# multiplefish/VPLines-SLAM

Hardware: AMD Instinct MI355X
Metric: sliding-window BA solves/sec (10 KF, 200 pts + 80 lines, 5 iters) (higher is better)
Workload: dtype f64

## Files before the change

vplines-slam_amd/csrc/ba_common.h:

```cpp
#pragma once
#include <hip/hip_runtime.h>
#include "ba_types.h"
#include "ba_asm_pattern.h"
#include "vpl_math.h"

namespace vpl {

#ifdef VPL_STAMPS
#define VPL_STAMP(B, w, i) do { if (threadIdx.x == 0) (B).dbg[(size_t)(w) * 64 + (i)] = (long long)__builtin_readcyclecounter(); } while (0)
#define VPL_IVAL(acc) long long acc = 0
#define VPL_IVAL_START(t) long long t = __builtin_readcyclecounter()
#define VPL_IVAL_ADD(acc, t) acc += __builtin_readcyclecounter() - (t)
#define VPL_IVAL_LAP(acc, t) do { const long long now_ = __builtin_readcyclecounter(); acc += now_ - (t); t = now_; } while (0)
#define VPL_IVAL_STORE(cond, dst, ...) do { long long* dst_ = (dst); if (dst_ && (cond)) { const long long v_[] = {__VA_ARGS__}; \
  for (int i_ = 0; i_ < (int)(sizeof(v_) / sizeof(v_[0])); ++i_) dst_[i_] = v_[i_]; } } while (0)
#else
#define VPL_STAMP(B, w, i) do {} while (0)
#define VPL_IVAL(acc) do {} while (0)
#define VPL_IVAL_START(t) do {} while (0)
#define VPL_IVAL_ADD(acc, t) do {} while (0)
#define VPL_IVAL_LAP(acc, t) do {} while (0)
#define VPL_IVAL_STORE(cond, dst, ...) do {} while (0)
#endif

__device__ __forceinline__ void count_active(const DevBatch& B, int k) {
  if (B.act && threadIdx.x == 0 && B.launch < ACT_SLOTS) atomicAdd(&B.act[4 * B.launch + k], 1);
}

__device__ __forceinline__ int ordered_window(const DevBatch& B) {
  const int w = B.ord_it == 0 ? (int)blockIdx.x : B.order[(size_t)(B.ord_it & 1) * B.nW + blockIdx.x];
  return __builtin_amdgcn_readfirstlane(w);
}

__device__ __forceinline__ double wave_sum(double v) {
#pragma unroll
  for (int o = 32; o > 0; o >>= 1) v += __shfl_xor(v, o, 64);
  return v;
}

template <int CTRL>
__device__ __forceinline__ double dpp_shr_f64(double v) {
  const int lo = __builtin_amdgcn_update_dpp(0, __double2loint(v), CTRL, 0xf, 0xf, true);
  const int hi = __builtin_amdgcn_update_dpp(0, __double2hiint(v), CTRL, 0xf, 0xf, true);
  return __hiloint2double(hi, lo);
}
__device__ __forceinline__ double row_sum16(double v) {
  v += dpp_shr_f64<0x111>(v);
  v += dpp_shr_f64<0x112>(v);
  v += dpp_shr_f64<0x114>(v);
  v += dpp_shr_f64<0x118>(v);
// ... 145 lines not shown
```

vplines-slam_amd/csrc/ba_limits.h:

```cpp
#pragma once

namespace vpl {

constexpr int NF = 11;
constexpr int NC = 171;
constexpr int NV = 72;
constexpr int MAXKEEP = 80;

}
```

vplines-slam_amd/csrc/ba_lin.h:

```cpp
#pragma once
#include "ba_common.h"

namespace vpl {

typedef double v4d_lin __attribute__((ext_vector_type(4)));
constexpr int LIN_THREADS = 512;
constexpr int STG_LD = 17;
constexpr int LIN_STAGE = 8 * 32 * STG_LD;
constexpr int PRE_LDS = 62;
constexpr int LIN_HW = 720;
constexpr int PREP_NMAX = 112;
__host__ __device__ constexpr int lin_stage_doubles(int maxL) {
  const int ln = 8 * LIN_HW + 38 * maxL;
  const int pt = LIN_STAGE + 78 * 36 + NV;
  const int m = ln > pt ? ln : pt;
  return m > 4650 + 3570 ? m : 4650 + 3570;
}
constexpr int PREP_THREADS = 640;
inline size_t prep_smem(int max_prior_n) {
  const int ns = max_prior_n < PREP_NMAX ? max_prior_n : PREP_NMAX;
  return (size_t)((PREP_THREADS / 64) * 675 + ns * ns + ns + 84) * sizeof(double);
}
constexpr size_t PREP_SMEM = (size_t)((PREP_THREADS / 64) * 675 + PREP_NMAX * PREP_NMAX + PREP_NMAX + 84) * sizeof(double);

// ... 388 lines not shown
        for (int c2 = 0; c2 <= a; ++c2, ++t) { Hl[4 * a + c2] = la[t]; Hl[4 * c2 + a] = la[t]; }
#pragma unroll
        for (int c2 = 0; c2 < 6; ++c2) B.Wl[(li * 4 + a) * WS + WS - 6 + c2] = la[14 + 6 * a + c2];
      }
    }
  }
  for (int e = tid; e < LIN_HW; e += T) {
    double v = 0.0;
#pragma unroll
    for (int q = 0; q < 8; ++q) v += lin_ln_Hw(imuJ, q)[e];
    if (e < 693) {
      const int f = e / 63, q = e - 63 * f;
      if (q < 21) {
        int a, c2;
        tri_decode(q, a, c2);
        Hv[hvi(6 * f + a, 6 * f + c2)] += v;
      } else if (q < 57) {
        const int a = (q - 21) / 6, c2 = (q - 21) % 6;
        Hv[hvi(66 + a, 6 * f + c2)] += v;
      } else {
        gv[6 * f + (q - 57)] += v;
      }
    } else if (e < 714) {
      int a, c2;
      tri_decode(e - 693, a, c2);
      Hv[hvi(66 + a, 66 + c2)] += v;
    } else {
      gv[66 + (e - 714)] += v;
    }
  }
}

template <int MODE>
__device__ __forceinline__ void lin_imu_raw(const DevBatch& B, const int w, const double* xp, const double* xs, const double* plds, double* imuJ, double* imur,
                                               int* imuact, double (&sa)[2][4]) {
  constexpr bool MARG = MODE != 0;
  constexpr bool PRIOR_ONLY = MODE == 2;
  const int tid = threadIdx.x, T = LIN_THREADS, lane = tid & 63;
  for (int i = tid; i < 4650; i += T) imuJ[i] = 0.0;
#pragma unroll
  for (int q = 0; q < 2; ++q) {
    const int f = (tid >> 6) + 8 * q;
    const double* S = B.pre[(size_t)w * NF + (f < 10 ? f : 0) + 1].sqrt_info;
#pragma unroll
    for (int ks = 0; ks < 4; ++ks) {
      const int k = 4 * ks + (lane >> 4), i = lane & 15;
      sa[q][ks] = (f < 10 && i < 15 && k < 15 && k >= i) ? S[i * 15 + k] : 0.0;
    }
  }
  __syncthreads();
  if ((tid & 63) < 10 && tid < 128) {
    const int f = tid & 63, j = f + 1;
    const DevPreint& dp = *(const DevPreint*)(plds + PRE_LDS * f);
    bool act = MARG ? (j == 1 && dp.sum_dt < 10.0) : !(dp.sum_dt > 10.0);
    if (PRIOR_ONLY) act = false;
    if (tid < 64) imuact[f] = act ? 1 : 0;
    if (act) {
      PreInt p = load_preint(dp);
      if (tid < 64) {
        imu_residual_raw(p, xp + 7 * (j - 1), xs + 9 * (j - 1), xp + 7 * j, xs + 9 * j, B.opt.g_norm, imur + 15 * f);
      } else {
        ImuJac JB = imu_jacobian_raw(p, xp + 7 * (j - 1), xs + 9 * (j - 1), xp + 7 * j, xs + 9 * j, B.opt.g_norm);
        imu_jac_dense(JB, imuJ + 450 * f);
      }
    }
  }
}
__device__ __forceinline__ void lin_asm_request(const DevBatch& B, int2 (&asmd)[LIN_ASM_PER_THREAD]) {
  const int tid = threadIdx.x, T = LIN_THREADS;
#pragma unroll
  for (int u = 0; u < LIN_ASM_PER_THREAD; ++u) {
    const int i = u * T + tid;
    asmd[u] = ((const int2*)B.asm_tab)[i < NZ_N ? i : 0];
  }
}
__device__ __forceinline__ void lin_imu_whiten(double* imuJ, double* imur, const int* imuact, const double (&sa)[2][4]) {
  const int tid = threadIdx.x, T = LIN_THREADS, lane = tid & 63;
  double* imuH = lin_imuH(imuJ);
  const int wvi = tid >> 6, m16 = lane & 15, kk = lane >> 4;
  v4d_lin cd[2] = {{0, 0, 0, 0}, {0, 0, 0, 0}};
  for (int i = tid; i < 120; i += T) imuH[i] = 0.0;
#pragma unroll
  for (int q = 0; q < 2; ++q) {
    const int f = wvi + 8 * q;
    if (f >= 10) break;
    double* J = imuJ + 450 * f;
    double* rr = imur + 15 * f;
    const bool on = imuact[f] != 0;
    v4d_lin jw[2] = {{0, 0, 0, 0}, {0, 0, 0, 0}};
#pragma unroll
    for (int ct = 0; ct < 2; ++ct) {
      const int c = 16 * ct + m16;
#pragma unroll
      for (int ks = 0; ks < 4; ++ks) {
        const int k = 4 * ks + kk;
        const double bv = k < 15 ? (c < 30 ? J[k * 30 + c] : (c == 30 ? rr[k] : 0.0)) : 0.0;
        jw[ct] = __builtin_amdgcn_mfma_f64_16x16x4f64(on ? sa[q][ks] : 0.0, bv, jw[ct], 0, 0, 0);
      }
    }
    __builtin_amdgcn_wave_barrier();
    if (on) {
#pragma unroll
      for (int ct = 0; ct < 2; ++ct) {
        const double vals[4] = {jw[ct].x, jw[ct].y, jw[ct].z, jw[ct].w};
        const int c = 16 * ct + m16;
#pragma unroll
        for (int v = 0; v < 4; ++v) {
          const int r = kk + 4 * v;
          if (r < 15) {
            if (c < 30) J[r * 30 + c] = vals[v];
            else if (c == 30) rr[r] = vals[v];
          }
        }
      }
    }
    __builtin_amdgcn_fence(__ATOMIC_RELEASE, "workgroup");
    __builtin_amdgcn_wave_barrier();
    __builtin_amdgcn_fence(__ATOMIC_ACQUIRE, "workgroup");
    v4d_lin c00 = {0, 0, 0, 0}, c10 = {0, 0, 0, 0}, c11 = {0, 0, 0, 0};
#pragma unroll
    for (int ks = 0; ks < 4; ++ks) {
      const int k = 4 * ks + kk;
      const double lo = k < 15 ? J[k * 30 + m16] : 0.0;
      const double hi = (k < 15 && m16 < 14) ? J[k * 30 + 16 + m16] : 0.0;
      c00 = __builtin_amdgcn_mfma_f64_16x16x4f64(lo, lo, c00, 0, 0, 0);
      c10 = __builtin_amdgcn_mfma_f64_16x16x4f64(hi, lo, c10, 0, 0, 0);
      c11 = __builtin_amdgcn_mfma_f64_16x16x4f64(hi, hi, c11, 0, 0, 0);
    }
    {
      const double v00[4] = {c00.x, c00.y, c00.z, c00.w}, v10[4] = {c10.x, c10.y, c10.z, c10.w}, v11[4] = {c11.x, c11.y, c11.z, c11.w};
      double keep[4] = {0, 0, 0, 0};
#pragma unroll
      for (int v = 0; v < 4; ++v) {
        const int i0 = kk + 4 * v, j0 = m16;
        if (i0 < 15 && j0 < 15) keep[v] = v00[v];
        const int i1 = 16 + kk + 4 * v;
        if (i1 < 30) {
          if (j0 < 15) imuH[11 * 120 + 225 * f + 15 * (i1 - 15) + j0] = v10[v];
          else imuH[120 * (f + 1) + (i1 - 15) * (i1 - 14) / 2 + 0] = v10[v];
          const int j1 = 16 + m16;
          if (j1 < 30 && j1 <= i1) imuH[120 * (f + 1) + (i1 - 15) * (i1 - 14) / 2 + (j1 - 15)] = v11[v];
        }
        if (i0 == 15) {
          if (j0 < 15) imuH[11 * 120 + 225 * f + j0] = v00[v];
          else imuH[120 * (f + 1)] = v00[v];
        }
      }
      cd[q] = v4d_lin{keep[0], keep[1], keep[2], keep[3]};
    }
  }
  __syncthreads();
#pragma unroll
  for (int q = 0; q < 2; ++q) {
    const int f = wvi + 8 * q;
    if (f >= 10) break;
    const double keep[4] = {cd[q].x, cd[q].y, cd[q].z, cd[q].w};
#pragma unroll
    for (int v = 0; v < 4; ++v) {
      const int i0 = kk + 4 * v, j0 = m16;
      if (i0 < 15 && j0 <= i0) imuH[120 * f + i0 * (i0 + 1) / 2 + j0] += keep[v];
    }
  }
}
__device__ __forceinline__ void lin_imu_cost(const double* imur, const int* imuact, double& cost) {
  const int tid = threadIdx.x;
  if (tid < 10 && imuact[tid]) {
    double s = 0;
    for (int k = 0; k < 15; ++k) s += imur[15 * tid + k] * imur[15 * tid + k];
    cost += 0.5 * s;
  }
}

__device__ __forceinline__ void lin_handover_in(const DevBatch& B, const int w, double* sm, double& cost) {
  const int tid = threadIdx.x, T = LIN_THREADS;
  if (tid == 0) {
    while (__hip_atomic_load(&B.lin_flag[w], __ATOMIC_RELAXED, __HIP_MEMORY_SCOPE_AGENT) != 1) __builtin_amdgcn_s_sleep(32);
    __hip_atomic_store(&B.lin_flag[w], 0, __ATOMIC_RELAXED, __HIP_MEMORY_SCOPE_AGENT);
  }
  __syncthreads();
  const double* part = B.lin_part + (size_t)w * LIN_PART;
  for (int i = tid; i < HV_DOUBLES + NV; i += T) sm[i] += __hip_atomic_load(&part[i], __ATOMIC_RELAXED, __HIP_MEMORY_SCOPE_AGENT);
  if (tid == 0) cost += __hip_atomic_load(&part[HV_DOUBLES + NV], __ATOMIC_RELAXED, __HIP_MEMORY_SCOPE_AGENT);
  __syncthreads();
}

__device__ __forceinline__ void lin_asm_store(const int2 d, const double* Hv, const double* imuH, const double* prH, const int* invmap,
                                                 const bool prior_lds, const bool ex_free, double* Hout) {
  const int hv = d.x & 0xffff, im = d.x >> 16, r = d.y & 255, c = (d.y >> 8) & 255, e = d.y >> 16;
  const double vh = Hv[hv ? hv - 1 : 0], vi = imuH[im ? im - 1 : 0];
  const int ir = prior_lds ? invmap[r] : -1, ic = prior_lds ? invmap[c] : -1;
  const bool hp = ir >= 0 && ic >= 0;
  const int hi_ = ic > ir ? ic : ir, lo_ = ic > ir ? ir : ic;
  const double vp = prH[hp ? hi_ * (hi_ + 1) / 2 + lo_ : 0];
  double v = hv ? vh : 0.0;
  v += im ? vi : 0.0;
// ... 439 lines not shown
          for (int a = 0; a < 6; ++a) {
            if (a >= c0) {
              const double gev = row_sum16(Je[a] * r[0] + Je[6 + a] * r[1]);
              if (leader) lds_add(&Hw[714 + a], gev);
            }
#pragma unroll
            for (int c2 = 0; c2 <= a; ++c2, ++t) {
              if (a < c0 || c2 < c0) continue;
              const double v = row_sum16(Je[a] * Je[c2] + Je[6 + a] * Je[6 + c2]);
              if (leader) lds_add(&Hw[693 + t], v);
            }
          }
        }
      }
      if (act) {
        double* Wl = B.Wl + li * 4 * WS;
#pragma unroll
        for (int a = 0; a < 4; ++a)
#pragma unroll
          for (int c2 = 0; c2 < 6; ++c2) Wl[a * WS + 6 * k + c2] = Wj[6 * a + c2];
      }
    }
  }
  __syncthreads();
  lin_lines_out(B, w, Hv, gv, imuJ, nL);
  __syncthreads();
  VPL_STAMP(B, w, 25);
  double sa[2][4];
  lin_imu_raw<MODE>(B, w, xp, xs, plds, imuJ, imur, imuact, sa);
  __syncthreads();
  VPL_STAMP(B, w, 28);
  int2 asmd[LIN_ASM_PER_THREAD];
  lin_asm_request(B, asmd);
  lin_imu_whiten(imuJ, imur, imuact, sa);
  __syncthreads();
  lin_imu_cost(imur, imuact, cost);
  if (ROLE == 2) {
    lin_handover_in(B, w, sm, cost);
  } else if (!MARG) {
    if (tid == 0) cost += cost_pts;
  }
  VPL_STAMP(B, w, 20);
  lin_assemble(B, w, Hv, gv, imuJ, imur, prg, prH, PRH_N, invmap, imuact, P.n, ex_free, asmd);
  VPL_STAMP(B, w, 21);
  lin_finish<MODE>(tr, red, cost);
}
template <int MODE>
__global__ __launch_bounds__(LIN_THREADS) void k_lin(DevBatch B) {
  extern __shared__ double sm[];
  lin_body<MODE, 0>(B, MODE == 0 ? ordered_window(B) : (int)blockIdx.x, sm);
}
__global__ __launch_bounds__(LIN_THREADS) void k_lin2(DevBatch B) {
  extern __shared__ double sm[];
  const int nlin = B.ord_it == 0 ? B.nW : B.ord_cnt[2 * (B.ord_it & 1)];
  if (2 * nlin > B.ncu) {
    if ((int)blockIdx.x < B.nW) lin_body<0, 0>(B, ordered_window(B), sm);
    return;
  }
  const int b = (int)(blockIdx.x >> 4) * 8 + (int)(blockIdx.x & 7);
  if (b >= B.nW) return;
  const int w = __builtin_amdgcn_readfirstlane(B.ord_it == 0 ? b : B.order[(size_t)(B.ord_it & 1) * B.nW + b]);
  if (blockIdx.x & 8) lin_body<0, 2>(B, w, sm);
  else lin_body<0, 1>(B, w, sm);
}

constexpr size_t LIN_LDS_BUDGET = 158 * 1024;
inline size_t lin_smem_base(int maxP, int maxL) {
// ... 17 lines not shown
```

vplines-slam_amd/csrc/vpl_math.h:

```cpp
#pragma once
#include <math.h>

#ifdef __HIPCC__
#define VPL_HD __host__ __device__ __forceinline__
#else
#define VPL_HD inline
#endif

namespace vpl {

struct V3 {
  double x, y, z;
};
struct M3 {
  double m[9];
};

VPL_HD V3 v3(double x, double y, double z) { return V3{x, y, z}; }
VPL_HD V3 operator+(V3 a, V3 b) { return V3{a.x + b.x, a.y + b.y, a.z + b.z}; }
VPL_HD V3 operator-(V3 a, V3 b) { return V3{a.x - b.x, a.y - b.y, a.z - b.z}; }
VPL_HD V3 operator-(V3 a) { return V3{-a.x, -a.y, -a.z}; }
VPL_HD V3 operator*(V3 a, double s) { return V3{a.x * s, a.y * s, a.z * s}; }
VPL_HD V3 operator*(double s, V3 a) { return V3{a.x * s, a.y * s, a.z * s}; }
VPL_HD double dot(V3 a, V3 b) { return a.x * b.x + a.y * b.y + a.z * b.z; }
// ... 393 lines not shown
};
VPL_HD void imu_residual_raw(const PreInt& p, const double* pi, const double* sbi, const double* pj, const double* sbj,
                             double g_norm, double* r) {
  V3 Pi{pi[0], pi[1], pi[2]}, Pj{pj[0], pj[1], pj[2]};
  Q4 Qi = qpose(pi), Qj = qpose(pj);
  V3 Vi{sbi[0], sbi[1], sbi[2]}, Bai{sbi[3], sbi[4], sbi[5]}, Bgi{sbi[6], sbi[7], sbi[8]};
  V3 Vj{sbj[0], sbj[1], sbj[2]}, Baj{sbj[3], sbj[4], sbj[5]}, Bgj{sbj[6], sbj[7], sbj[8]};
  V3 G{0, 0, g_norm};
  V3 dba = Bai - p.lba, dbg = Bgi - p.lbg;
  Q4 cq = qmul(p.dq, deltaQ(mul(p.dq_dbg, dbg)));
  V3 cv = p.dv + mul(p.dv_dba, dba) + mul(p.dv_dbg, dbg);
  V3 cp = p.dp + mul(p.dp_dba, dba) + mul(p.dp_dbg, dbg);
  double dt = p.sum_dt;
  Q4 Qii = qinv(Qi);
  V3 rp = qrot(Qii, G * (0.5 * dt * dt) + Pj - Pi - Vi * dt) - cp;
  Q4 qe = qmul(qinv(cq), qmul(Qii, Qj));
  V3 rq{2 * qe.x, 2 * qe.y, 2 * qe.z};
  V3 rv = qrot(Qii, G * dt + Vj - Vi) - cv;
  V3 rba = Baj - Bai, rbg = Bgj - Bgi;
  r[0] = rp.x; r[1] = rp.y; r[2] = rp.z; r[3] = rq.x; r[4] = rq.y; r[5] = rq.z;
  r[6] = rv.x; r[7] = rv.y; r[8] = rv.z; r[9] = rba.x; r[10] = rba.y; r[11] = rba.z;
  r[12] = rbg.x; r[13] = rbg.y; r[14] = rbg.z;
}
VPL_HD M3 qleft_br(Q4 q) {
  M3 S = skew(V3{q.x, q.y, q.z});
  S.m[0] += q.w; S.m[4] += q.w; S.m[8] += q.w;
  return S;
}
VPL_HD M3 qright_br(Q4 q) {
  M3 S = skew(V3{-q.x, -q.y, -q.z});
  S.m[0] += q.w; S.m[4] += q.w; S.m[8] += q.w;
  return S;
}
struct ImuJac {
  M3 pi_pp, pi_pr, pi_rr, pi_vr;
  M3 si_pv, si_pba, si_pbg, si_rbg, si_vv, si_vba, si_vbg;
  M3 pj_pp, pj_rr;
  M3 sj_vv;
};
VPL_HD M3 neg(const M3& A) {
  M3 C;
#pragma unroll
  for (int k = 0; k < 9; ++k) C.m[k] = -A.m[k];
  return C;
}
VPL_HD M3 scale(const M3& A, double s) {
  M3 C;
#pragma unroll
  for (int k = 0; k < 9; ++k) C.m[k] = A.m[k] * s;
  return C;
}
VPL_HD ImuJac imu_jacobian_raw(const PreInt& p, const double* pi, const double* sbi, const double* pj,
                               const double* sbj, double g_norm) {
  V3 Pi{pi[0], pi[1], pi[2]}, Pj{pj[0], pj[1], pj[2]};
  Q4 Qi = qpose(pi), Qj = qpose(pj);
  V3 Vi{sbi[0], sbi[1], sbi[2]}, Bgi{sbi[6], sbi[7], sbi[8]};
  V3 Vj{sbj[0], sbj[1], sbj[2]};
  V3 G{0, 0, g_norm};
  double dt = p.sum_dt;
  Q4 Qii = qinv(Qi);
  M3 RiT = qmat(Qii);
  Q4 cq = qmul(p.dq, deltaQ(mul(p.dq_dbg, Bgi - p.lbg)));
  ImuJac J;
  J.pi_pp = neg(RiT);
  J.pi_pr = skew(qrot(Qii, G * (0.5 * dt * dt) + Pj - Pi - Vi * dt));
  {
    Q4 ql = qmul(qinv(Qj), Qi);
    M3 A = qleft_br(ql), B = qright_br(cq);
    M3 AB = mul(A, B);
    V3 vl{ql.x, ql.y, ql.z}, vr{cq.x, cq.y, cq.z};
    double vlv[3] = {vl.x, vl.y, vl.z}, vrv[3] = {vr.x, vr.y, vr.z};
#pragma unroll
    for (int i = 0; i < 3; ++i)
#pragma unroll
      for (int j = 0; j < 3; ++j) AB.m[3 * i + j] += -vlv[i] * vrv[j];
    J.pi_rr = neg(AB);
  }
  J.pi_vr = skew(qrot(Qii, G * dt + Vj - Vi));
  J.si_pv = scale(RiT, -dt);
  J.si_pba = neg(p.dp_dba);
  J.si_pbg = neg(p.dp_dbg);
  J.si_rbg = neg(mul(qleft_br(qmul(qmul(qinv(Qj), Qi), cq)), p.dq_dbg));
  J.si_vv = neg(RiT);
  J.si_vba = neg(p.dv_dba);
  J.si_vbg = neg(p.dv_dbg);
  J.pj_pp = RiT;
  J.pj_rr = qleft_br(qmul(qmul(qinv(cq), Qii), Qj));
  J.sj_vv = RiT;
  return J;
}
VPL_HD void put33(double* J, int ld, int r0, int c0, const M3& B) {
#pragma unroll
  for (int i = 0; i < 3; ++i)
#pragma unroll
    for (int j = 0; j < 3; ++j) J[(r0 + i) * ld + c0 + j] = B.m[3 * i + j];
}
VPL_HD void imu_jac_dense(const ImuJac& B, double* J ) {
  put33(J, 30, 0, 0, B.pi_pp); put33(J, 30, 0, 3, B.pi_pr); put33(J, 30, 3, 3, B.pi_rr); put33(J, 30, 6, 3, B.pi_vr);
  put33(J, 30, 0, 6, B.si_pv); put33(J, 30, 0, 9, B.si_pba); put33(J, 30, 0, 12, B.si_pbg);
  put33(J, 30, 3, 12, B.si_rbg);
  put33(J, 30, 6, 6, B.si_vv); put33(J, 30, 6, 9, B.si_vba); put33(J, 30, 6, 12, B.si_vbg);
  J[9 * 30 + 9] = -1; J[10 * 30 + 10] = -1; J[11 * 30 + 11] = -1;
  J[12 * 30 + 12] = -1; J[13 * 30 + 13] = -1; J[14 * 30 + 14] = -1;
  put33(J, 30, 0, 15, B.pj_pp); put33(J, 30, 3, 18, B.pj_rr);
  put33(J, 30, 6, 21, B.sj_vv);
  J[9 * 30 + 24] = 1; J[10 * 30 + 25] = 1; J[11 * 30 + 26] = 1;
  J[12 * 30 + 27] = 1; J[13 * 30 + 28] = 1; J[14 * 30 + 29] = 1;
}

}
```

vplines-slam_amd/csrc/vplines_ba.hip:

```cpp
#include <hip/hip_runtime.h>

#include <algorithm>
#include <chrono>
#include <memory>
#include <cstdlib>
#include <cstring>
#include <string>
#include <vector>

#include "vplines_ba.h"
#include "ba_types.h"
#include "ba_lin.h"
#include "ba_pack.h"
#include "ba_solve.h"
#include "ba_step.h"
#include "ba_marg.h"
#include "ba_prior_eig.h"
#include "ba_lineopt.h"
#include "ba_factors.h"
#include "ba_odo.h"
#include "odo_tracks.h"
#include "host_common.h"

using namespace vpl;
// ... 87 lines not shown
  {
    int ncu = 0;
    if (hipDeviceGetAttribute(&ncu, hipDeviceAttributeMultiprocessorCount, device) != hipSuccess || ncu <= 0) ncu = 256;
    if (const char* sv = std::getenv("VPL_BA_LIN_SPLIT")) ncu = std::atoi(sv) ? 1 << 30 : 0;
    B.ncu = ncu;
  }
  B.maxPR = max_point_unit_rounds(B.maxP, B.maxPO);
  B.maxKS = max_schur_ksteps(B.maxP, B.maxL);
  B.llSlots = line_lane_slots(B.maxL);
  const size_t W = max_windows;
  hipError_t e = hipSuccess;
#define AL(ptr, n) if (e == hipSuccess) e = dalloc(c, &B.ptr, (size_t)(n))
  AL(pose, W * 77); AL(sb, W * 99); AL(ex, W * 7); AL(invd, W * B.maxP); AL(orth, W * B.maxL * 4);
  AL(pose_c, W * 77); AL(sb_c, W * 99); AL(ex_c, W * 7); AL(invd_c, W * B.maxP); AL(orth_c, W * B.maxL * 4); AL(lw, W * B.maxL * 6); AL(lw_c, W * B.maxL * 6);
  AL(lin_part, W * LIN_PART); AL(lin_pcost, W); AL(lin_flag, W);
  AL(pose_0, W * 77); AL(sb_0, W * 99); AL(ex_0, W * 7); AL(invd_0, W * B.maxP); AL(plk_0, W * B.maxL * 6);
  AL(plk, W * B.maxL * 6); AL(gauge, W * 4); AL(fail_ref, W * 13); AL(orth_in, W);
  AL(nP, W); AL(nL, W);
  AL(pt_start, W * B.maxP); AL(pt_nobs, W * B.maxP); AL(pt_off, W * B.maxP); AL(pt_obs, W * B.maxPO * 3);
  AL(ps_list, W * B.maxP); AL(ps_cnt, W * (NF + 1)); AL(pu_lane, W * B.maxPR * 1024); AL(pu_sub, W * B.maxPR * 512); AL(pu_cnt, W); AL(pu_cnt0, W);
  AL(ln_start, W * B.maxL); AL(ln_nobs, W * B.maxL); AL(ln_off, W * B.maxL); AL(ln_obs, W * B.maxLO * 8);
  AL(nLO, W); AL(lo_ln, W * B.maxLO);
  AL(ll_tab, W * B.llSlots * 2); AL(ll_np, W);
  AL(pre, W * NF);
  AL(pr_n, W); AL(pr_nb, W); AL(pr_kind, W * MAXPB); AL(pr_frame, W * MAXPB); AL(pr_idx, W * MAXPB);
  AL(pr_x0, W * MAXPB * 9); AL(pr_J0, W * MAXPN * MAXPN); AL(pr_r0, W * MAXPN); AL(pr_H, W * MAXPN * MAXPN); AL(pr_g0, W * MAXPN);
  AL(pr_map, W * MAXPN);
  AL(Hcc, W * NCP); AL(gc, W * NC); AL(asm_tab, 2 * NCP); AL(Hpp, W * B.maxP); AL(gp, W * B.maxP); AL(Wp, W * B.maxP * NV);
  AL(Hll, W * B.maxL * 16); AL(gl, W * B.maxL * 4); AL(Wl, W * B.maxL * 4 * NV); AL(lchol, W * B.maxL * 10);
  AL(tr, W);
  AL(scale, W * B.nfull); AL(diag, W * B.nfull); AL(grad, W * B.nfull); AL(gn, W * B.nfull);
  AL(mg_n, W); AL(mg_nb, W); AL(mg_kind, W * MAXPB); AL(mg_frame, W * MAXPB); AL(mg_idx, W * MAXPB);
  AL(mg_cam, W * MAXPB); AL(mg_x0, W * MAXPB * 9); AL(mg_J0, W * MAXKEEP * MAXKEEP); AL(mg_r0, W * MAXKEEP);
  AL(mg_A, W * MAXKEEP * MAXKEEP); AL(mg_b, W * MAXKEEP); AL(mg_m, W); AL(dbg, W * 64); AL(ln_removed, W * B.maxL); AL(ln_tri, W * B.maxL);
  if (e == hipSuccess) e = dalloc(c, &c->d_act, (size_t)ACT_SLOTS * 4);
  AL(order, 2 * W); AL(ord_cnt, 4);
  AL(sk_tab, W * B.maxKS * 4); AL(sk_wave, W * 8 * SK_WSTRIDE); AL(sacc, W * SACC_N); AL(nz_tab, NZ_N); AL(ycs, W * 176); AL(sx, W * 8); AL(path, W);
#undef AL
  if (e != hipSuccess) return VPL_E_HIP;
  if (lin_smem_base(c->maxP, c->maxL) > LIN_LDS_BUDGET) return VPL_E_CAPACITY;
  B.prhN = lin_prh_n(c->maxP, c->maxL);
  {
    std::vector<int> nz, tab;
    asm_build_tables(nz, tab);
    if ((int)nz.size() != NZ_N || (int)tab.size() != 2 * NCP) return VPL_E_HIP;
    if (hipMemcpy(B.asm_tab, tab.data(), tab.size() * sizeof(int), hipMemcpyHostToDevice) != hipSuccess) return VPL_E_HIP;
    if (hipMemcpy(B.nz_tab, nz.data(), nz.size() * sizeof(int), hipMemcpyHostToDevice) != hipSuccess) return VPL_E_HIP;
  }
  static size_t lin_max = 0, solve_max = 0, schur_max = 0, back_max = 0, step_max = 0;
  lin_max = std::max(lin_max, lin_smem(c->maxP, c->maxL));
  solve_max = std::max(solve_max, solve_smem(c->maxP, c->maxL));
  schur_max = std::max(schur_max, schur_smem(c->maxP, c->maxL));
  back_max = std::max(back_max, back_smem(c->maxP, c->maxL));
  step_max = std::max(step_max, step_smem(c->maxP, c->maxL));
  if (schur_max > 159 * 1024 || back_max > 159 * 1024) return VPL_E_CAPACITY;
  const std::pair<const void*, size_t> lds[] = {
      {(const void*)k_lin2, lin_max}, {(const void*)k_lin<1>, lin_max}, {(const void*)k_lin<2>, lin_max},
      {(const void*)k_solve, solve_max}, {(const void*)k_schur<3>, schur_max}, {(const void*)k_schur<5>, schur_max},
      {(const void*)k_schur_mixed, schur_max}, {(const void*)k_chol, chol_smem()}, {(const void*)k_back, back_max},
      {(const void*)k_step<3, false>, step_max}, {(const void*)k_step<3, true>, step_max}, {(const void*)k_step<5, false>, step_max},
      {(const void*)k_prep, PREP_SMEM}, {(const void*)k_marg<MARG_THREADS>, MARG_LDS_MAX}, {(const void*)k_marg<256>, MARG_LDS_SMALL},
      {(const void*)k_prior_eigen, prior_eig_layout(MAXKEEP).bytes}, {(const void*)k_init_align, init_lds_bytes(INIT_NMAX)}};
  for (const auto& k : lds)
    if (hipFuncSetAttribute(k.first, hipFuncAttributeMaxDynamicSharedMemorySize, (int)k.second) != hipSuccess) return VPL_E_HIP;
  vpl_ba_default_options(&c->opt);
  if (const char* gv = std::getenv("VPL_BA_GRAPH")) c->use_graph = std::atoi(gv) != 0;
  if (const char* gv = std::getenv("VPL_BA_GENERAL")) c->force_general = std::atoi(gv) != 0;
// ... 921 lines not shown
  HIPCHK(c, dat.alloc(N * 8)); HIPCHK(c, drt.alloc(N * 8)); HIPCHK(c, drank.alloc(N * 4)); HIPCHK(c, dperm.alloc(N * MAXKEEP * 4));
  HIPCHK(c, dJ.alloc(N * M2 * 8)); HIPCHK(c, dr.alloc(N * MAXKEEP * 8));
  HIPCHK(c, hipMemcpyAsync(dn.p, n, N * 4, hipMemcpyHostToDevice, c->stream));
  HIPCHK(c, hipMemcpyAsync(dA.p, A, N * M2 * 8, hipMemcpyHostToDevice, c->stream));
  HIPCHK(c, hipMemcpyAsync(db.p, b, N * MAXKEEP * 8, hipMemcpyHostToDevice, c->stream));
  HIPCHK(c, hipMemcpyAsync(dat.p, abs_tol, N * 8, hipMemcpyHostToDevice, c->stream));
  HIPCHK(c, hipMemcpyAsync(drt.p, rel_tol, N * 8, hipMemcpyHostToDevice, c->stream));
  HIPCHK(c, hipMemsetAsync(drank.p, 0xff, N * 4, c->stream));
  HIPCHK(c, hipMemsetAsync(dperm.p, 0xff, N * MAXKEEP * 4, c->stream));
  HIPCHK(c, hipMemsetAsync(dJ.p, 0xff, N * M2 * 8, c->stream));
  HIPCHK(c, hipMemsetAsync(dr.p, 0xff, N * MAXKEEP * 8, c->stream));
  const size_t smem = (size_t)psd_test_lds_doubles(nmax) * sizeof(double);
  const void* kern = threads == 256 ? (const void*)k_psd_factor<256> : (const void*)k_psd_factor<512>;
  HIPCHK(c, hipFuncSetAttribute(kern, hipFuncAttributeMaxDynamicSharedMemorySize, psd_test_lds_doubles(MAXKEEP) * (int)sizeof(double)));
  if (threads == 256)
    hipLaunchKernelGGL(k_psd_factor<256>, dim3(n_cases), dim3(256), smem, c->stream, form, (const int*)dn.p, dA.d(), db.d(), dat.d(),
                       drt.d(), (int*)drank.p, (int*)dperm.p, dJ.d(), dr.d());
  else
    hipLaunchKernelGGL(k_psd_factor<512>, dim3(n_cases), dim3(512), smem, c->stream, form, (const int*)dn.p, dA.d(), db.d(), dat.d(),
                       drt.d(), (int*)drank.p, (int*)dperm.p, dJ.d(), dr.d());
  HIPCHK(c, hipGetLastError());
  HIPCHK(c, hipMemcpyAsync(rank, drank.p, N * 4, hipMemcpyDeviceToHost, c->stream));
  HIPCHK(c, hipMemcpyAsync(perm, dperm.p, N * MAXKEEP * 4, hipMemcpyDeviceToHost, c->stream));
  HIPCHK(c, hipMemcpyAsync(J0, dJ.p, N * M2 * 8, hipMemcpyDeviceToHost, c->stream));
  HIPCHK(c, hipMemcpyAsync(r0, dr.p, N * MAXKEEP * 8, hipMemcpyDeviceToHost, c->stream));
  HIPCHK(c, hipStreamSynchronize(c->stream));
  return VPL_OK;
}

int vpl_ba_debug_guards(vpl_ctx* c) { return debug_guards(c); }
int vpl_ba_debug_allocs(vpl_ctx* c, long long* n_arrays, long long* payload_bytes) { return debug_allocs(c, n_arrays, payload_bytes); }

int vpl_ba_debug_stamps(vpl_ctx* c, int w, long long* out) {
  HIPCHK(c, hipMemcpy(out, c->B.dbg + (size_t)w * 64, 64 * 8, hipMemcpyDeviceToHost));
  return VPL_OK;
}

int vpl_ba_debug_point_units(int n_points, const int* point_start, const int* point_nobs, int max_rounds, int* lane_table,
                             int* unit_table, int* rounds, int* rounds0) {
  if (n_points < 0 || !point_start || !point_nobs || !lane_table || !unit_table || !rounds || !rounds0 || max_rounds < 1) return VPL_E_INVALID;
  std::vector<int> off(n_points + 1, 0), list(n_points + 1, 0);
  int cnt[NF + 1];
  int o = 0;
  for (int p = 0; p < n_points; ++p) {
    if (point_start[p] < 0 || point_nobs[p] < 2 || point_start[p] + point_nobs[p] > NF) return VPL_E_INVALID;
    off[p] = o; o += point_nobs[p];
  }
  sort_points_by_start(n_points, point_start, point_nobs, list.data(), cnt);
  PointUnitLayout PL;
  if (!pack_point_units(point_nobs, off.data(), list.data(), cnt, max_rounds, lane_table, unit_table, &PL)) return VPL_E_CAPACITY;
  *rounds = PL.rounds; *rounds0 = PL.rounds0;
  return VPL_OK;
}
int vpl_ba_debug_point_chains(const int* unit_table, int rounds, int rounds0, int marg_pass) {
  if (!unit_table || rounds < 0 || rounds0 < 0 || rounds0 > rounds) return VPL_E_INVALID;
  PointUnitLayout PL;
  PL.rounds = rounds; PL.rounds0 = rounds0;
  return point_unit_chains_finish(unit_table, PL, marg_pass != 0) ? 1 : 0;
}

int vpl_ba_enable_kernel_timing(vpl_ctx* c, int enable) {
  if (!c) return VPL_E_INVALID;
  c->timing = enable != 0;
  c->ktimes.clear();
  return VPL_OK;
}
int vpl_ba_kernel_times(vpl_ctx* c, int* count, const char** names, double* total_ms, int* launches) {
// ... 34 lines not shown
```

Measured before the change: 273,800.

## Split IMU Jacobian into per-wave groups and rebalance IMU whitening across waves

Splits the IMU Jacobian computation into four independent block groups, each computed by a different wave alongside the residual wave, instead of one thread per frame computing the whole Jacobian. It also reorganises IMU whitening and Gram products so that eight waves each own one frame and the remaining frames are dealt out across waves by tile. Zeroing of the IMU Hessian is restricted to inactive frames. The intent is to shorten the serial per-thread Jacobian latency and balance MFMA work across waves, at the cost of recomputing shared quaternion terms in each group and adding an extra block barrier. Extra debug stamp slots are added as well.

```diff
diff --git a/vplines-slam_amd/csrc/ba_common.h b/vplines-slam_amd/csrc/ba_common.h
--- a/vplines-slam_amd/csrc/ba_common.h
+++ b/vplines-slam_amd/csrc/ba_common.h
@@ -7,7 +7,8 @@
 namespace vpl {
 
 #ifdef VPL_STAMPS
-#define VPL_STAMP(B, w, i) do { if (threadIdx.x == 0) (B).dbg[(size_t)(w) * 64 + (i)] = (long long)__builtin_readcyclecounter(); } while (0)
+#define VPL_STAMP_T(B, w, i, t) do { if (threadIdx.x == (t)) (B).dbg[(size_t)(w) * DBG_SLOTS + (i)] = (long long)__builtin_readcyclecounter(); } while (0)
+#define VPL_STAMP(B, w, i) VPL_STAMP_T(B, w, i, 0)
 #define VPL_IVAL(acc) long long acc = 0
 #define VPL_IVAL_START(t) long long t = __builtin_readcyclecounter()
 #define VPL_IVAL_ADD(acc, t) acc += __builtin_readcyclecounter() - (t)
@@ -16,6 +17,7 @@
   for (int i_ = 0; i_ < (int)(sizeof(v_) / sizeof(v_[0])); ++i_) dst_[i_] = v_[i_]; } } while (0)
 #else
 #define VPL_STAMP(B, w, i) do {} while (0)
+#define VPL_STAMP_T(B, w, i, t) do {} while (0)
 #define VPL_IVAL(acc) do {} while (0)
 #define VPL_IVAL_START(t) do {} while (0)
 #define VPL_IVAL_ADD(acc, t) do {} while (0)
diff --git a/vplines-slam_amd/csrc/ba_limits.h b/vplines-slam_amd/csrc/ba_limits.h
--- a/vplines-slam_amd/csrc/ba_limits.h
+++ b/vplines-slam_amd/csrc/ba_limits.h
@@ -5,6 +5,7 @@
 constexpr int NF = 11;
 constexpr int NC = 171;
 constexpr int NV = 72;
+constexpr int DBG_SLOTS = 80;
 constexpr int MAXKEEP = 80;
 
 }
diff --git a/vplines-slam_amd/csrc/ba_lin.h b/vplines-slam_amd/csrc/ba_lin.h
--- a/vplines-slam_amd/csrc/ba_lin.h
+++ b/vplines-slam_amd/csrc/ba_lin.h
@@ -444,39 +444,60 @@
 }
 
 template <int MODE>
+__device__ __forceinline__ bool lin_imu_active(const double* plds, const int f) {
+  const DevPreint& dp = *(const DevPreint*)(plds + PRE_LDS * f);
+  if (MODE == 2) return false;
+  return MODE != 0 ? (f == 0 && dp.sum_dt < 10.0) : !(dp.sum_dt > 10.0);
+}
+template <int MODE>
+struct LinImuDeal {
+  static constexpr int OWN = MODE == 0 ? 8 : 0;
+  static constexpr int DEALT = MODE == 0 ? 2 : (MODE == 1 ? 1 : 0);
+};
+template <int MODE>
+__device__ __forceinline__ void lin_imu_request(const DevBatch& B, const int w, const double* plds, const int q, const int wvi, double (&sa)[4]) {
+  using D = LinImuDeal<MODE>;
+  const int lane = threadIdx.x & 63;
+  const int f = q == 0 ? wvi : D::OWN + (wvi >> 1);
+  const bool have = q == 0 ? wvi < D::OWN : wvi < 2 * D::DEALT;
+  const bool on = have && lin_imu_active<MODE>(plds, have ? f : 0);
+  const double* S = B.pre[(size_t)w * NF + (have ? f : 0) + 1].sqrt_info;
+#pragma unroll
+  for (int ks = 0; ks < 4; ++ks) {
+    const int k = 4 * ks + (lane >> 4), i = lane & 15;
+    sa[ks] = (on && i < 15 && k < 15 && k >= i) ? S[i * 15 + k] : 0.0;
+  }
+}
+template <int MODE>
 __device__ __forceinline__ void lin_imu_raw(const DevBatch& B, const int w, const double* xp, const double* xs, const double* plds, double* imuJ, double* imur,
                                                int* imuact, double (&sa)[2][4]) {
-  constexpr bool MARG = MODE != 0;
-  constexpr bool PRIOR_ONLY = MODE == 2;
   const int tid = threadIdx.x, T = LIN_THREADS, lane = tid & 63;
+  const int wvi = __builtin_amdgcn_readfirstlane(tid >> 6);
   for (int i = tid; i < 4650; i += T) imuJ[i] = 0.0;
-#pragma unroll
-  for (int q = 0; q < 2; ++q) {
-    const int f = (tid >> 6) + 8 * q;
-    const double* S = B.pre[(size_t)w * NF + (f < 10 ? f : 0) + 1].sqrt_info;
-#pragma unroll
-    for (int ks = 0; ks < 4; ++ks) {
-      const int k = 4 * ks + (lane >> 4), i = lane & 15;
-      sa[q][ks] = (f < 10 && i < 15 && k < 15 && k >= i) ? S[i * 15 + k] : 0.0;
-    }
-  }
-  __syncthreads();
-  if ((tid & 63) < 10 && tid < 128) {
-    const int f = tid & 63, j = f + 1;
-    const DevPreint& dp = *(const DevPreint*)(plds + PRE_LDS * f);
-    bool act = MARG ? (j == 1 && dp.sum_dt < 10.0) : !(dp.sum_dt > 10.0);
-    if (PRIOR_ONLY) act = false;
-    if (tid < 64) imuact[f] = act ? 1 : 0;
+  lin_imu_request<MODE>(B, w, plds, 0, wvi, sa[0]);
+  lin_imu_request<MODE>(B, w, plds, 1, wvi, sa[1]);
+  __syncthreads();
+  VPL_STAMP(B, w, 64);
+  if (lane < 10 && wvi < 5) {
+    const int f = lane, j = f + 1;
+    const bool act = lin_imu_active<MODE>(plds, f);
+    if (wvi == 0) imuact[f] = act ? 1 : 0;
     if (act) {
-      PreInt p = load_preint(dp);
-      if (tid < 64) {
-        imu_residual_raw(p, xp + 7 * (j - 1), xs + 9 * (j - 1), xp + 7 * j, xs + 9 * j, B.opt.g_norm, imur + 15 * f);
-      } else {
-        ImuJac JB = imu_jacobian_raw(p, xp + 7 * (j - 1), xs + 9 * (j - 1), xp + 7 * j, xs + 9 * j, B.opt.g_norm);
-        imu_jac_dense(JB, imuJ + 450 * f);
-      }
-    }
-  }
+      const DevPreint& dp = *(const DevPreint*)(plds + PRE_LDS * f);
+      const double *pi = xp + 7 * (j - 1), *sbi = xs + 9 * (j - 1), *pj = xp + 7 * j, *sbj = xs + 9 * j;
+      const double g_norm = B.opt.g_norm;
+      if (wvi == 0) { const PreInt p = load_preint(dp); imu_residual_raw(p, pi, sbi, pj, sbj, g_norm, imur + 15 * f); }
+      else if (wvi == 1) { const PreInt p = load_preint(dp); imu_jac_group_dense(0, p, pi, sbi, pj, sbj, g_norm, imuJ + 450 * f); }
+      else if (wvi == 2) { const PreInt p = load_preint(dp); imu_jac_group_dense(1, p, pi, sbi, pj, sbj, g_norm, imuJ + 450 * f); }
+      else if (wvi == 3) { const PreInt p = load_preint(dp); imu_jac_group_dense(2, p, pi, sbi, pj, sbj, g_norm, imuJ + 450 * f); }
+      else { const PreInt p = load_preint(dp); imu_jac_group_dense(3, p, pi, sbi, pj, sbj, g_norm, imuJ + 450 * f); }
+    }
+  }
+  VPL_STAMP(B, w, 65);
+  VPL_STAMP_T(B, w, 72, 64);
+  VPL_STAMP_T(B, w, 73, 128);
+  VPL_STAMP_T(B, w, 74, 192);
+  VPL_STAMP_T(B, w, 75, 256);
 }
 __device__ __forceinline__ void lin_asm_request(const DevBatch& B, int2 (&asmd)[LIN_ASM_PER_THREAD]) {
   const int tid = threadIdx.x, T = LIN_THREADS;
@@ -486,46 +507,89 @@
     asmd[u] = ((const int2*)B.asm_tab)[i < NZ_N ? i : 0];
   }
 }
-__device__ __forceinline__ void lin_imu_whiten(double* imuJ, double* imur, const int* imuact, const double (&sa)[2][4]) {
+__device__ __forceinline__ v4d_lin lin_imu_whiten_tile(const double* J, const double* rr, const double (&sa)[4], const int ct, const int m16, const int kk) {
+  v4d_lin jw = {0, 0, 0, 0};
+  const int c = 16 * ct + m16;
+#pragma unroll
+  for (int ks = 0; ks < 4; ++ks) {
+    const int k = 4 * ks + kk;
+    const double bv = k < 15 ? (c < 30 ? J[k * 30 + c] : (c == 30 ? rr[k] : 0.0)) : 0.0;
+    jw = __builtin_amdgcn_mfma_f64_16x16x4f64(sa[ks], bv, jw, 0, 0, 0);
+  }
+  return jw;
+}
+__device__ __forceinline__ void lin_imu_whiten_store(double* J, double* rr, const v4d_lin jw, const int ct, const int m16, const int kk) {
+  const double vals[4] = {jw.x, jw.y, jw.z, jw.w};
+  const int c = 16 * ct + m16;
+#pragma unroll
+  for (int v = 0; v < 4; ++v) {
+    const int r = kk + 4 * v;
+    if (r < 15) {
+      if (c < 30) J[r * 30 + c] = vals[v];
+      else if (c == 30) rr[r] = vals[v];
+    }
+  }
+}
+__device__ __forceinline__ v4d_lin lin_imu_put00(double* imuH, const int f, const v4d_lin c00, const int m16, const int kk) {
+  const double v00[4] = {c00.x, c00.y, c00.z, c00.w};
+  double keep[4] = {0, 0, 0, 0};
+#pragma unroll
+  for (int v = 0; v < 4; ++v) {
+    const int i0 = kk + 4 * v, j0 = m16;
+    if (i0 < 15 && j0 < 15) keep[v] = v00[v];
+    if (i0 == 15) {
+      if (j0 < 15) imuH[11 * 120 + 225 * f + j0] = v00[v];
+      else imuH[120 * (f + 1)] = v00[v];
+    }
+  }
+  return v4d_lin{keep[0], keep[1], keep[2], keep[3]};
+}
+__device__ __forceinline__ void lin_imu_put10(double* imuH, const int f, const v4d_lin c10, const int m16, const int kk) {
+  const double v10[4] = {c10.x, c10.y, c10.z, c10.w};
+#pragma unroll
+  for (int v = 0; v < 4; ++v) {
+    const int i1 = 16 + kk + 4 * v, j0 = m16;
+    if (i1 < 30) {
+      if (j0 < 15) imuH[11 * 120 + 225 * f + 15 * (i1 - 15) + j0] = v10[v];
+      else imuH[120 * (f + 1) + (i1 - 15) * (i1 - 14) / 2 + 0] = v10[v];
+    }
+  }
+}
+__device__ __forceinline__ void lin_imu_put11(double* imuH, const int f, const v4d_lin c11, const int m16, const int kk) {
+  const double v11[4] = {c11.x, c11.y, c11.z, c11.w};
+#pragma unroll
+  for (int v = 0; v < 4; ++v) {
+    const int i1 = 16 + kk + 4 * v, j1 = 16 + m16;
+    if (i1 < 30 && j1 < 30 && j1 <= i1) imuH[120 * (f + 1) + (i1 - 15) * (i1 - 14) / 2 + (j1 - 15)] = v11[v];
+  }
+}
+__device__ __forceinline__ void lin_imu_add_kept(double* imuH, const int f, const v4d_lin cd, const int m16, const int kk) {
+  const double keep[4] = {cd.x, cd.y, cd.z, cd.w};
+#pragma unroll
+  for (int v = 0; v < 4; ++v) {
+    const int i0 = kk + 4 * v, j0 = m16;
+    if (i0 < 15 && j0 <= i0) imuH[120 * f + i0 * (i0 + 1) / 2 + j0] += keep[v];
+  }
+}
+template <int MODE>
+__device__ __forceinline__ void lin_imu_whiten(const DevBatch& B, const int w, double* imuJ, double* imur, const int* imuact, const double (&sa)[2][4]) {
+  using D = LinImuDeal<MODE>;
   const int tid = threadIdx.x, T = LIN_THREADS, lane = tid & 63;
   double* imuH = lin_imuH(imuJ);
-  const int wvi = tid >> 6, m16 = lane & 15, kk = lane >> 4;
+  const int wvi = __builtin_amdgcn_readfirstlane(tid >> 6), m16 = lane & 15, kk = lane >> 4;
+  for (int i = tid; i < 11 * 120 + 10 * 225; i += T) {
+    const int f = i < 11 * 120 ? i / 120 - 1 : (i - 11 * 120) / 225;
+    if (f < 0 || imuact[f] == 0) imuH[i] = 0.0;
+  }
   v4d_lin cd[2] = {{0, 0, 0, 0}, {0, 0, 0, 0}};
-  for (int i = tid; i < 120; i += T) imuH[i] = 0.0;
-#pragma unroll
-  for (int q = 0; q < 2; ++q) {
-    const int f = wvi + 8 * q;
-    if (f >= 10) break;
+  if (D::OWN > 0 && wvi < D::OWN && imuact[wvi] != 0) {
+    const int f = wvi;
     double* J = imuJ + 450 * f;
     double* rr = imur + 15 * f;
-    const bool on = imuact[f] != 0;
-    v4d_lin jw[2] = {{0, 0, 0, 0}, {0, 0, 0, 0}};
-#pragma unroll
-    for (int ct = 0; ct < 2; ++ct) {
-      const int c = 16 * ct + m16;
-#pragma unroll
-      for (int ks = 0; ks < 4; ++ks) {
-        const int k = 4 * ks + kk;
-        const double bv = k < 15 ? (c < 30 ? J[k * 30 + c] : (c == 30 ? rr[k] : 0.0)) : 0.0;
-        jw[ct] = __builtin_amdgcn_mfma_f64_16x16x4f64(on ? sa[q][ks] : 0.0, bv, jw[ct], 0, 0, 0);
-      }
-    }
+    const v4d_lin jw0 = lin_imu_whiten_tile(J, rr, sa[0], 0, m16, kk), jw1 = lin_imu_whiten_tile(J, rr, sa[0], 1, m16, kk);
     __builtin_amdgcn_wave_barrier();
-    if (on) {
-#pragma unroll
-      for (int ct = 0; ct < 2; ++ct) {
-        const double vals[4] = {jw[ct].x, jw[ct].y, jw[ct].z, jw[ct].w};
-        const int c = 16 * ct + m16;
-#pragma unroll
-        for (int v = 0; v < 4; ++v) {
-          const int r = kk + 4 * v;
-          if (r < 15) {
-            if (c < 30) J[r * 30 + c] = vals[v];
-            else if (c == 30) rr[r] = vals[v];
-          }
-        }
-      }
-    }
+    lin_imu_whiten_store(J, rr, jw0, 0, m16, kk);
+    lin_imu_whiten_store(J, rr, jw1, 1, m16, kk);
     __builtin_amdgcn_fence(__ATOMIC_RELEASE, "workgroup");
     __builtin_amdgcn_wave_barrier();
     __builtin_amdgcn_fence(__ATOMIC_ACQUIRE, "workgroup");
@@ -539,40 +603,46 @@
       c10 = __builtin_amdgcn_mfma_f64_16x16x4f64(hi, lo, c10, 0, 0, 0);
       c11 = __builtin_amdgcn_mfma_f64_16x16x4f64(hi, hi, c11, 0, 0, 0);
     }
-    {
-      const double v00[4] = {c00.x, c00.y, c00.z, c00.w}, v10[4] = {c10.x, c10.y, c10.z, c10.w}, v11[4] = {c11.x, c11.y, c11.z, c11.w};
-      double keep[4] = {0, 0, 0, 0};
-#pragma unroll
-      for (int v = 0; v < 4; ++v) {
-        const int i0 = kk + 4 * v, j0 = m16;
-        if (i0 < 15 && j0 < 15) keep[v] = v00[v];
-        const int i1 = 16 + kk + 4 * v;
-        if (i1 < 30) {
-          if (j0 < 15) imuH[11 * 120 + 225 * f + 15 * (i1 - 15) + j0] = v10[v];
-          else imuH[120 * (f + 1) + (i1 - 15) * (i1 - 14) / 2 + 0] = v10[v];
-          const int j1 = 16 + m16;
-          if (j1 < 30 && j1 <= i1) imuH[120 * (f + 1) + (i1 - 15) * (i1 - 14) / 2 + (j1 - 15)] = v11[v];
-        }
-        if (i0 == 15) {
-          if (j0 < 15) imuH[11 * 120 + 225 * f + j0] = v00[v];
-          else imuH[120 * (f + 1)] = v00[v];
-        }
-      }
-      cd[q] = v4d_lin{keep[0], keep[1], keep[2], keep[3]};
-    }
-  }
-  __syncthreads();
-#pragma unroll
-  for (int q = 0; q < 2; ++q) {
-    const int f = wvi + 8 * q;
-    if (f >= 10) break;
-    const double keep[4] = {cd[q].x, cd[q].y, cd[q].z, cd[q].w};
-#pragma unroll
-    for (int v = 0; v < 4; ++v) {
-      const int i0 = kk + 4 * v, j0 = m16;
-      if (i0 < 15 && j0 <= i0) imuH[120 * f + i0 * (i0 + 1) / 2 + j0] += keep[v];
-    }
-  }
+    cd[0] = lin_imu_put00(imuH, f, c00, m16, kk);
+    lin_imu_put10(imuH, f, c10, m16, kk);
+    lin_imu_put11(imuH, f, c11, m16, kk);
+  }
+  VPL_STAMP(B, w, 68);
+  const int fj = D::OWN + wvi / 3, tj = wvi - 3 * (wvi / 3);
+  const bool dealt_j = D::DEALT > 0 && wvi < 3 * D::DEALT && imuact[wvi < 3 * D::DEALT ? fj : 0] != 0;
+  if (D::DEALT > 0) {
+    const int fw = D::OWN + (wvi >> 1);
+    if (wvi < 2 * D::DEALT && imuact[wvi < 2 * D::DEALT ? fw : 0] != 0) {
+      double* J = imuJ + 450 * fw;
+      double* rr = imur + 15 * fw;
+      const v4d_lin jw = lin_imu_whiten_tile(J, rr, sa[1], wvi & 1, m16, kk);
+      __builtin_amdgcn_wave_barrier();
+      lin_imu_whiten_store(J, rr, jw, wvi & 1, m16, kk);
+    }
+    VPL_STAMP(B, w, 69);
+    __syncthreads();
+    VPL_STAMP(B, w, 76);
+    if (dealt_j) {
+      const double* J = imuJ + 450 * fj;
+      v4d_lin c = {0, 0, 0, 0};
+#pragma unroll
+      for (int ks = 0; ks < 4; ++ks) {
+        const int k = 4 * ks + kk;
+        const double lo = k < 15 ? J[k * 30 + m16] : 0.0;
+        const double hi = (k < 15 && m16 < 14) ? J[k * 30 + 16 + m16] : 0.0;
+        c = __builtin_amdgcn_mfma_f64_16x16x4f64(tj == 0 ? lo : hi, tj == 2 ? hi : lo, c, 0, 0, 0);
+      }
+      if (tj == 0) cd[1] = lin_imu_put00(imuH, fj, c, m16, kk);
+      else if (tj == 1) lin_imu_put10(imuH, fj, c, m16, kk);
+      else lin_imu_put11(imuH, fj, c, m16, kk);
+    }
+    VPL_STAMP(B, w, 77);
+  }
+  __syncthreads();
+  VPL_STAMP(B, w, 70);
+  if (D::OWN > 0 && wvi < D::OWN) lin_imu_add_kept(imuH, wvi, cd[0], m16, kk);
+  if (dealt_j && tj == 0) lin_imu_add_kept(imuH, fj, cd[1], m16, kk);
+  VPL_STAMP(B, w, 71);
 }
 __device__ __forceinline__ void lin_imu_cost(const double* imur, const int* imuact, double& cost) {
   const int tid = threadIdx.x;
@@ -1078,7 +1148,7 @@
   VPL_STAMP(B, w, 28);
   int2 asmd[LIN_ASM_PER_THREAD];
   lin_asm_request(B, asmd);
-  lin_imu_whiten(imuJ, imur, imuact, sa);
+  lin_imu_whiten<MODE>(B, w, imuJ, imur, imuact, sa);
   __syncthreads();
   lin_imu_cost(imur, imuact, cost);
   if (ROLE == 2) {
diff --git a/vplines-slam_amd/csrc/vpl_math.h b/vplines-slam_amd/csrc/vpl_math.h
--- a/vplines-slam_amd/csrc/vpl_math.h
+++ b/vplines-slam_amd/csrc/vpl_math.h
@@ -449,12 +449,21 @@
   S.m[0] += q.w; S.m[4] += q.w; S.m[8] += q.w;
   return S;
 }
-struct ImuJac {
-  M3 pi_pp, pi_pr, pi_rr, pi_vr;
-  M3 si_pv, si_pba, si_pbg, si_rbg, si_vv, si_vba, si_vbg;
-  M3 pj_pp, pj_rr;
-  M3 sj_vv;
-};
+enum ImuJacBlock {
+  IJ_PI_PP, IJ_PI_PR, IJ_PI_RR, IJ_PI_VR,
+  IJ_SI_PV, IJ_SI_PBA, IJ_SI_PBG, IJ_SI_RBG, IJ_SI_VV, IJ_SI_VBA, IJ_SI_VBG,
+  IJ_PJ_PP, IJ_PJ_RR,
+  IJ_SJ_VV,
+  IJ_N
+};
+VPL_HD int imu_jac_row(int b) {
+  return (b == IJ_PI_RR || b == IJ_SI_RBG || b == IJ_PJ_RR) ? 3 : (b == IJ_PI_VR || b == IJ_SI_VV || b == IJ_SI_VBA || b == IJ_SI_VBG || b == IJ_SJ_VV) ? 6 : 0;
+}
+VPL_HD int imu_jac_col(int b) {
+  return b == IJ_PI_PP ? 0 : b <= IJ_PI_VR ? 3 : (b == IJ_SI_PV || b == IJ_SI_VV) ? 6 : (b == IJ_SI_PBA || b == IJ_SI_VBA) ? 9 : b <= IJ_SI_VBG ? 12
+       : b == IJ_PJ_PP ? 15 : b == IJ_PJ_RR ? 18 : 21;
+}
+struct ImuJac { M3 b[IJ_N]; };
 VPL_HD M3 neg(const M3& A) {
   M3 C;
 #pragma unroll
@@ -467,62 +476,104 @@
   for (int k = 0; k < 9; ++k) C.m[k] = A.m[k] * s;
   return C;
 }
-VPL_HD ImuJac imu_jacobian_raw(const PreInt& p, const double* pi, const double* sbi, const double* pj,
-                               const double* sbj, double g_norm) {
+VPL_HD void put33(double* J, int ld, int r0, int c0, const M3& B) {
+#pragma unroll
+  for (int i = 0; i < 3; ++i)
+#pragma unroll
+    for (int j = 0; j < 3; ++j) J[(r0 + i) * ld + c0 + j] = B.m[3 * i + j];
+}
+struct ImuJacToBlocks {
+  ImuJac* B;
+  VPL_HD void operator()(int b, const M3& M) const { B->b[b] = M; }
+};
+struct ImuJacToDense {
+  double* J;
+  VPL_HD void operator()(int b, const M3& M) const { put33(J, 30, imu_jac_row(b), imu_jac_col(b), M); }
+};
+template <class Put>
+VPL_HD void imu_jac_group0(const PreInt& p, const double* pi, const double* sbi, const double* pj, const double* sbj, double g_norm, const Put& put) {
   V3 Pi{pi[0], pi[1], pi[2]}, Pj{pj[0], pj[1], pj[2]};
-  Q4 Qi = qpose(pi), Qj = qpose(pj);
-  V3 Vi{sbi[0], sbi[1], sbi[2]}, Bgi{sbi[6], sbi[7], sbi[8]};
+  Q4 Qi = qpose(pi);
+  V3 Vi{sbi[0], sbi[1], sbi[2]};
   V3 Vj{sbj[0], sbj[1], sbj[2]};
   V3 G{0, 0, g_norm};
   double dt = p.sum_dt;
   Q4 Qii = qinv(Qi);
   M3 RiT = qmat(Qii);
+  put(IJ_PI_PP, neg(RiT));
+  put(IJ_PI_PR, skew(qrot(Qii, G * (0.5 * dt * dt) + Pj - Pi - Vi * dt)));
+  put(IJ_PI_VR, skew(qrot(Qii, G * dt + Vj - Vi)));
+  put(IJ_SI_PV, scale(RiT, -dt));
+  put(IJ_SI_VV, neg(RiT));
+  put(IJ_PJ_PP, RiT);
+  put(IJ_SJ_VV, RiT);
+}
+VPL_HD Q4 imu_corrected_dq(const PreInt& p, const double* sbi) {
+  V3 Bgi{sbi[6], sbi[7], sbi[8]};
   Q4 cq = qmul(p.dq, deltaQ(mul(p.dq_dbg, Bgi - p.lbg)));
-  ImuJac J;
-  J.pi_pp = neg(RiT);
-  J.pi_pr = skew(qrot(Qii, G * (0.5 * dt * dt) + Pj - Pi - Vi * dt));
-  {
-    Q4 ql = qmul(qinv(Qj), Qi);
-    M3 A = qleft_br(ql), B = qright_br(cq);
-    M3 AB = mul(A, B);
-    V3 vl{ql.x, ql.y, ql.z}, vr{cq.x, cq.y, cq.z};
-    double vlv[3] = {vl.x, vl.y, vl.z}, vrv[3] = {vr.x, vr.y, vr.z};
-#pragma unroll
-    for (int i = 0; i < 3; ++i)
-#pragma unroll
-      for (int j = 0; j < 3; ++j) AB.m[3 * i + j] += -vlv[i] * vrv[j];
-    J.pi_rr = neg(AB);
-  }
-  J.pi_vr = skew(qrot(Qii, G * dt + Vj - Vi));
-  J.si_pv = scale(RiT, -dt);
-  J.si_pba = neg(p.dp_dba);
-  J.si_pbg = neg(p.dp_dbg);
-  J.si_rbg = neg(mul(qleft_br(qmul(qmul(qinv(Qj), Qi), cq)), p.dq_dbg));
-  J.si_vv = neg(RiT);
-  J.si_vba = neg(p.dv_dba);
-  J.si_vbg = neg(p.dv_dbg);
-  J.pj_pp = RiT;
-  J.pj_rr = qleft_br(qmul(qmul(qinv(cq), Qii), Qj));
-  J.sj_vv = RiT;
-  return J;
-}
-VPL_HD void put33(double* J, int ld, int r0, int c0, const M3& B) {
+  return cq;
+}
+template <class Put>
+VPL_HD void imu_jac_group1(const PreInt& p, const double* pi, const double* sbi, const double* pj, const Put& put) {
+  Q4 Qi = qpose(pi), Qj = qpose(pj);
+  Q4 cq = imu_corrected_dq(p, sbi);
+  Q4 ql = qmul(qinv(Qj), Qi);
+  M3 A = qleft_br(ql), B = qright_br(cq);
+  M3 AB = mul(A, B);
+  V3 vl{ql.x, ql.y, ql.z}, vr{cq.x, cq.y, cq.z};
+  double vlv[3] = {vl.x, vl.y, vl.z}, vrv[3] = {vr.x, vr.y, vr.z};
 #pragma unroll
   for (int i = 0; i < 3; ++i)
 #pragma unroll
-    for (int j = 0; j < 3; ++j) J[(r0 + i) * ld + c0 + j] = B.m[3 * i + j];
-}
-VPL_HD void imu_jac_dense(const ImuJac& B, double* J ) {
-  put33(J, 30, 0, 0, B.pi_pp); put33(J, 30, 0, 3, B.pi_pr); put33(J, 30, 3, 3, B.pi_rr); put33(J, 30, 6, 3, B.pi_vr);
-  put33(J, 30, 0, 6, B.si_pv); put33(J, 30, 0, 9, B.si_pba); put33(J, 30, 0, 12, B.si_pbg);
-  put33(J, 30, 3, 12, B.si_rbg);
-  put33(J, 30, 6, 6, B.si_vv); put33(J, 30, 6, 9, B.si_vba); put33(J, 30, 6, 12, B.si_vbg);
+    for (int j = 0; j < 3; ++j) AB.m[3 * i + j] += -vlv[i] * vrv[j];
+  put(IJ_PI_RR, neg(AB));
+}
+template <class Put>
+VPL_HD void imu_jac_group2(const PreInt& p, const double* pi, const double* sbi, const double* pj, const Put& put) {
+  Q4 Qi = qpose(pi), Qj = qpose(pj);
+  Q4 cq = imu_corrected_dq(p, sbi);
+  put(IJ_SI_RBG, neg(mul(qleft_br(qmul(qmul(qinv(Qj), Qi), cq)), p.dq_dbg)));
+}
+template <class Put>
+VPL_HD void imu_jac_group3(const PreInt& p, const double* pi, const double* sbi, const double* pj, const Put& put) {
+  Q4 Qi = qpose(pi), Qj = qpose(pj);
+  Q4 Qii = qinv(Qi);
+  Q4 cq = imu_corrected_dq(p, sbi);
+  put(IJ_PJ_RR, qleft_br(qmul(qmul(qinv(cq), Qii), Qj)));
+  put(IJ_SI_PBA, neg(p.dp_dba));
+  put(IJ_SI_PBG, neg(p.dp_dbg));
+  put(IJ_SI_VBA, neg(p.dv_dba));
+  put(IJ_SI_VBG, neg(p.dv_dbg));
+}
+VPL_HD void imu_jac_ones(double* J ) {
   J[9 * 30 + 9] = -1; J[10 * 30 + 10] = -1; J[11 * 30 + 11] = -1;
   J[12 * 30 + 12] = -1; J[13 * 30 + 13] = -1; J[14 * 30 + 14] = -1;
-  put33(J, 30, 0, 15, B.pj_pp); put33(J, 30, 3, 18, B.pj_rr);
-  put33(J, 30, 6, 21, B.sj_vv);
   J[9 * 30 + 24] = 1; J[10 * 30 + 25] = 1; J[11 * 30 + 26] = 1;
   J[12 * 30 + 27] = 1; J[13 * 30 + 28] = 1; J[14 * 30 + 29] = 1;
 }
-
-}
+VPL_HD void imu_jac_group_dense(int q, const PreInt& p, const double* pi, const double* sbi, const double* pj, const double* sbj, double g_norm,
+                                double* J ) {
+  const ImuJacToDense put{J};
+  if (q == 0) imu_jac_group0(p, pi, sbi, pj, sbj, g_norm, put);
+  else if (q == 1) imu_jac_group1(p, pi, sbi, pj, put);
+  else if (q == 2) imu_jac_group2(p, pi, sbi, pj, put);
+  else { imu_jac_group3(p, pi, sbi, pj, put); imu_jac_ones(J); }
+}
+VPL_HD ImuJac imu_jacobian_raw(const PreInt& p, const double* pi, const double* sbi, const double* pj,
+                               const double* sbj, double g_norm) {
+  ImuJac J;
+  const ImuJacToBlocks put{&J};
+  imu_jac_group0(p, pi, sbi, pj, sbj, g_norm, put);
+  imu_jac_group1(p, pi, sbi, pj, put);
+  imu_jac_group2(p, pi, sbi, pj, put);
+  imu_jac_group3(p, pi, sbi, pj, put);
+  return J;
+}
+VPL_HD void imu_jac_dense(const ImuJac& B, double* J ) {
+  const ImuJacToDense put{J};
+#pragma unroll
+  for (int b = 0; b < IJ_N; ++b) put(b, B.b[b]);
+  imu_jac_ones(J);
+}
+
+}
diff --git a/vplines-slam_amd/csrc/vplines_ba.hip b/vplines-slam_amd/csrc/vplines_ba.hip
--- a/vplines-slam_amd/csrc/vplines_ba.hip
+++ b/vplines-slam_amd/csrc/vplines_ba.hip
@@ -143,7 +143,7 @@
   AL(scale, W * B.nfull); AL(diag, W * B.nfull); AL(grad, W * B.nfull); AL(gn, W * B.nfull);
   AL(mg_n, W); AL(mg_nb, W); AL(mg_kind, W * MAXPB); AL(mg_frame, W * MAXPB); AL(mg_idx, W * MAXPB);
   AL(mg_cam, W * MAXPB); AL(mg_x0, W * MAXPB * 9); AL(mg_J0, W * MAXKEEP * MAXKEEP); AL(mg_r0, W * MAXKEEP);
-  AL(mg_A, W * MAXKEEP * MAXKEEP); AL(mg_b, W * MAXKEEP); AL(mg_m, W); AL(dbg, W * 64); AL(ln_removed, W * B.maxL); AL(ln_tri, W * B.maxL);
+  AL(mg_A, W * MAXKEEP * MAXKEEP); AL(mg_b, W * MAXKEEP); AL(mg_m, W); AL(dbg, W * DBG_SLOTS); AL(ln_removed, W * B.maxL); AL(ln_tri, W * B.maxL);
   if (e == hipSuccess) e = dalloc(c, &c->d_act, (size_t)ACT_SLOTS * 4);
   AL(order, 2 * W); AL(ord_cnt, 4);
   AL(sk_tab, W * B.maxKS * 4); AL(sk_wave, W * 8 * SK_WSTRIDE); AL(sacc, W * SACC_N); AL(nz_tab, NZ_N); AL(ycs, W * 176); AL(sx, W * 8); AL(path, W);
@@ -1131,7 +1131,7 @@
 int vpl_ba_debug_allocs(vpl_ctx* c, long long* n_arrays, long long* payload_bytes) { return debug_allocs(c, n_arrays, payload_bytes); }
 
 int vpl_ba_debug_stamps(vpl_ctx* c, int w, long long* out) {
-  HIPCHK(c, hipMemcpy(out, c->B.dbg + (size_t)w * 64, 64 * 8, hipMemcpyDeviceToHost));
+  HIPCHK(c, hipMemcpy(out, c->B.dbg + (size_t)w * DBG_SLOTS, DBG_SLOTS * 8, hipMemcpyDeviceToHost));
   return VPL_OK;
 }
 
```

Result: no change. 276,500 (median of 6 runs) (+1.0%).
